# ekzhu/datasketch

Measured on AMD Instinct MI355X. Metric: MinHash signatures/sec (1M sets x 256 tokens, num_perm=128), higher is better.
Workload: dtype u64

## Files before the change

### datasketch_amd/csrc/mhx_internal.h

```cpp
#pragma once

#include <hip/hip_runtime.h>

#include <algorithm>
#include <cstdarg>
#include <cstdint>
#include <cstdio>
#include <mutex>
#include <string>
#include <unordered_map>

#include "mhx.h"

namespace mhx {

void set_error(const char *fmt, ...);
int fail(int code, const char *fmt, ...);
void forgive();

#define MHX_HIP_CHECK(expr)                                                                      \
    do {                                                                                         \
        hipError_t _e = (expr);                                                                  \
        if (_e != hipSuccess) {                                                                  \
            return ::mhx::fail(_e == hipErrorOutOfMemory ? MHX_ERR_OOM : MHX_ERR_HIP,            \
                               "%s failed: %s (%s:%d)", #expr, hipGetErrorString(_e), __FILE__,  \
                               __LINE__);                                                        \
        }                                                                                        \
    } while (0)

constexpr int kSigDigests = 2;
constexpr int kSigDigestsBM = 3;
constexpr int32_t kWeightedRows = -2;

constexpr unsigned int kPairListCap = 16384;
constexpr size_t kWorkBytes = 64 + sizeof(unsigned int) * kPairListCap;

#define MHX_GUARD(ctxp) std::lock_guard<std::recursive_mutex> _mhx_guard((ctxp)->mu)

#define MHX_REQUIRE(cond, ...)                                       \
    do {                                                             \
        if (!(cond)) return ::mhx::fail(MHX_ERR_INVALID, __VA_ARGS__); \
    } while (0)

hipError_t dev_malloc(void **p, size_t bytes, bool caller = false);
hipError_t dev_free(void *p);
bool guard_mode();

}

struct mhx_ctx {
    std::recursive_mutex mu;
    int device = 0;
    hipStream_t stream = nullptr;
    int num_cus = 0;
    int hw_cus = 0;
    int64_t lds_per_block = 64 << 10;
    int64_t hbm_bytes = 0;
    char name[128] = {0};
    void *scratch[5] = {nullptr, nullptr, nullptr, nullptr, nullptr};
    size_t scratch_bytes[5] = {0, 0, 0, 0, 0};
    int64_t opt_minhash_path = 0;
    int64_t opt_minhash_packed = 0;
    int64_t opt_minhash_adapt = 0;
    int64_t opt_minhash_share = 0;
    int64_t opt_minhash_p3 = 0;
    int64_t opt_minhash_ties = 0;
    int64_t opt_minhash_split = 0;
    int64_t opt_blocks_per_cu = 0;
    int64_t opt_debug_cus = 0;
    int64_t opt_minhash_prefetch = 1;
    int64_t opt_minhash_alias = -1;
    int64_t opt_weighted_path = 0;
    int64_t opt_weighted_min_dim = 0;
    int64_t opt_weighted_rescue = 0;
    int64_t opt_weighted_plan = 0;
    int64_t opt_weighted_kernel = 0;
    int64_t opt_weighted_debug = 0;
    int64_t opt_weighted_split = 0;
    int64_t opt_weighted_tail = 0;
    int64_t opt_weighted_direct = 0;
    int64_t opt_lsh_sort = 0;
    int64_t opt_lsh_gather = 0;
    int64_t opt_lsh_sort_bits = 0;
    int64_t opt_lsh_prehash = 0;
    int64_t opt_lsh_chunk = 0;
    int64_t opt_lsh_bigbins = 0;
    int64_t opt_lsh_team = 0;
    int64_t opt_lsh_merge_items = 0;
    int64_t opt_lsh_levels = 0;
    int64_t opt_pack_fused = 0;
    int64_t opt_weighted_refill = 0;
    int64_t opt_hll_split_tokens = 0;
    int64_t opt_bloom_lanes = 0;
    int64_t opt_jaccard_topk_path = 0;
    int64_t opt_jaccard_topk_segments = 0;
    int64_t opt_overlap_bins = 0;
    int64_t opt_host_chunk_bytes = 0;

    hipStream_t copy_in = nullptr;
    hipStream_t copy_out = nullptr;
    int ensure_copy_streams();

    unsigned long long *d_stats = nullptr;
    uint8_t *d_redo = nullptr;
    int64_t redo_capacity = 0;
    int64_t redo_sets = 0;
    int ensure_redo(int64_t n_sets);
    unsigned int *d_work = nullptr;
    int ensure_work();

    int ensure_scratch(int slot, size_t bytes);
    int activate() const;
};

struct mhx_perm {
    mhx_ctx *ctx = nullptr;
    int32_t num_perm = 0;
    uint64_t *d_a = nullptr;
    uint64_t *d_b = nullptr;
};

struct mhx_wgen {
    mhx_ctx *ctx = nullptr;
    int32_t sample_size = 0;
    int32_t dim = 0;
    float *d_params = nullptr;
    int32_t s_pad = 0;
    bool table_fast = false;
    float *d_aos = nullptr;
    float *d_walk_a = nullptr;
    uint32_t *d_walk_c = nullptr;
    void *d_walk_plan = nullptr;
    int plan_index = 0;
    bool walk_ok = false;
};

struct mhx_event {
    mhx_ctx *ctx = nullptr;
    hipEvent_t ev = nullptr;
};

namespace mhx {

int launch_minhash_bulk(mhx_perm *perm, const void *d_hv, int hv_dtype, const int64_t *d_offsets,
                        int64_t fixed_len, int64_t n_sets, int64_t total_tokens,
                        const uint64_t *d_init, int64_t init_stride, void *d_out, int out_dtype,
                        int64_t first_token = 0);
int launch_sha1_tokens(mhx_ctx *ctx, const uint8_t *d_bytes, const int64_t *d_offsets, int64_t n_tokens,
                       int out_dtype, void *d_out);
int launch_sha1_windows(mhx_ctx *ctx, const uint8_t *d_bytes, const int64_t *d_item_offsets, const int64_t *d_doc_offsets,
                        const int64_t *d_set_offsets, int64_t n_docs, int64_t n_windows, int64_t width, int out_dtype, void *d_out);
int launch_xxh_tokens(mhx_ctx *ctx, const uint8_t *d_bytes, const int64_t *d_offsets, int64_t n_tokens, int out_dtype, void *d_out);
int launch_xxh_windows(mhx_ctx *ctx, const uint8_t *d_bytes, const int64_t *d_item_offsets, const int64_t *d_doc_offsets,
                       const int64_t *d_set_offsets, int64_t n_docs, int64_t n_windows, int64_t width, int out_dtype, void *d_out);
int launch_words_count(mhx_ctx *ctx, const uint8_t *d_bytes, int64_t n_bytes, const int64_t *d_doc_offsets, int64_t n_docs,
                       const uint8_t *table, int64_t *n_words, int64_t *n_out_bytes);
int launch_words_emit(mhx_ctx *ctx, const uint8_t *d_bytes, int64_t n_bytes, const int64_t *d_doc_offsets, int64_t n_docs,
                      const uint8_t *table, uint8_t *d_out, int64_t *d_item_offsets, int64_t *d_word_doc_offsets);
int launch_minhash_merge(mhx_ctx *ctx, const uint64_t *d_x, const uint64_t *d_y, int64_t count,
                         uint64_t *d_out);
int launch_weighted(mhx_wgen *gen, const int64_t *d_indptr, const int32_t *d_indices,
                    const float *d_values, int values_are_logs, int64_t n_rows, int64_t nnz,
                    int64_t *d_out, uint8_t *d_nonempty);
int launch_weighted_log(mhx_ctx *ctx, const float *d_x, int64_t n, float *d_out);
int launch_wgen_transpose(mhx_wgen *gen, const float *d_rs, const float *d_lncs, const float *d_betas);
int launch_bbit_pack(mhx_ctx *ctx, const void *d_sig, int sig_dtype, int64_t n, int32_t k, int32_t b,
                     uint64_t *d_out);
int launch_band_keys(mhx_ctx *ctx, const uint64_t *d_sig, int64_t n, int32_t k, int32_t bands,
                     int32_t r, uint64_t *d_out);
int launch_band_digests(mhx_ctx *ctx, const void *d_sig, int sig_dtype, int64_t n, int32_t k, int32_t bands, int32_t r,
                        uint64_t *d_out, int layout = 0);
int launch_bbit_digest_fused(mhx_ctx *ctx, const void *d_sig, int sig_dtype, int64_t n, int32_t k, int32_t b, int32_t bands,
                             int32_t r, uint64_t *d_blocks, uint64_t *d_digests, int layout, bool *done);
int launch_jaccard_pairs(mhx_ctx *ctx, const void *d_a, const void *d_b, int sig_dtype, int32_t k, const int64_t *d_pairs,
                         int64_t m, int32_t *d_counts);
int launch_weighted_jaccard_pairs(mhx_ctx *ctx, const void *d_a, const void *d_b, int32_t samples, const int64_t *d_pairs, int64_t m,
                                  int32_t *d_counts);
int launch_weighted_dense(mhx_wgen *gen, const float *d_x, int values_are_logs, int64_t n_rows, int64_t *d_out,
                          uint8_t *d_nonempty);
int launch_lsh_candidate_pairs(mhx_ctx *ctx, const uint64_t *d_sorted_digests, const uint32_t *d_sorted_rows, int64_t n,
                               int32_t bands, int64_t *d_pairs, int64_t capacity, int64_t *n_pairs, int64_t *n_raw);
int launch_lsh_sort_bands(mhx_ctx *ctx, const void *d_sig, int sig_dtype, int64_t n, int32_t k, int32_t bands, int32_t r,
                          uint64_t *d_sorted_digests, uint32_t *d_sorted_rows);
int launch_lsh_query(mhx_ctx *ctx, const uint64_t *d_sorted_digests, const uint32_t *d_sorted_rows, int64_t n, int32_t bands,
                     int32_t r, const void *d_q_sig, const void *d_idx_sig, int sig_dtype, int32_t k, int64_t m,
                     int64_t *d_pairs, int64_t capacity, int64_t *n_pairs);
int launch_lsh_ensemble_query(mhx_ctx *ctx, const mhx_ensemble_level *levels, int32_t n_levels, const int64_t *start, int32_t n_parts,
                              const void *d_idx_sig, int sig_dtype, int32_t k, const void *d_q_sig, int64_t m, const uint8_t *d_choice,
// ... 69 lines not shown
```

### datasketch_amd/csrc/minhash_kernels.hip

```cpp
#include <type_traits>

#include "mhx_internal.h"

namespace mhx {
namespace {

constexpr uint64_t kMersenne = (1ull << 61) - 1;
constexpr uint32_t kMaxHash = 0xFFFFFFFFu;
constexpr int kWave = 64;

struct BulkArgs {
    const void *hv;
    const int64_t *offsets;
    int64_t fixed_len;
    int64_t n_sets;
    const uint64_t *a;
    const uint64_t *b;
    int32_t num_perm;
    int32_t path;
    unsigned long long *stats;
    uint8_t *redo;
    int32_t redo_match;
    unsigned int *sieve_hint;
    unsigned int *mode_word;
// ... 682 lines not shown
    const int lane = threadIdx.x & (kWave - 1);
    const TokT MHX_CONST_AS *hv = as_const(hv_vec);
    Perms<P> pm, pm_biased;
    bool active[P];
#pragma unroll
    for (int p = 0; p < P; ++p) {
        const int k = kbase + p * kWave + lane;
        active[p] = k < num_perm;
        const uint64_t av = active[p] ? a[k] : 0;
        pm.a_lo[p] = pm_biased.a_lo[p] = (uint32_t)av;
        pm.a_hi[p] = pm_biased.a_hi[p] = (uint32_t)(av >> 32);
        pm.b[p] = active[p] ? b[k] : 0;
        pm_biased.b[p] = pm.b[p] + 1;
    }
    Minima<P> res;
    bool redo = exact_only;
    if (!exact_only) {
        uint32_t acc[P];
#pragma unroll
        for (int p = 0; p < P; ++p) acc[p] = kMaxHash;
        hash_range<P, false, TokT>(hv, beg, end, pm_biased, acc);
        bool suspicious = false;
#pragma unroll
        for (int p = 0; p < P; ++p) {
            suspicious |= active[p] && acc[p] <= 7u;
            res.v[p] = acc[p] - 1u;
        }
        redo = __any(suspicious);
    }
    if (redo) {
        if (!exact_only && stats && lane == 0) atomicAdd(stats + 1, 1ull);
#pragma unroll
        for (int p = 0; p < P; ++p) res.v[p] = kMaxHash;
        hash_range<P, true, TokT>(hv, beg, end, pm, res.v);
    }
    return res;
}

template <int P, typename TokT, bool TAIL = true, bool TIES = false, bool SHARE = false, bool SHORT = true>
__device__ __forceinline__ bool sieve_minima(const TokT MHX_CONST_AS *hv, const TokT *hv_vec, int64_t beg,
                                             int64_t end, const Perms<P> &pm, const Perms<P> &pm_biased,
                                             const SievePerms<P> &sp, unsigned long long *stats, int lane,
                                             uint32_t *lds, uint32_t (&res)[P], bool *tied = nullptr) {
    const int64_t n = end - beg;
    const int nrows = (int)min(n / kRowTokens, (int64_t)(1 << 27));
#pragma unroll
    for (int p = 0; p < P; ++p) res[p] = kMaxHash;
    bool bad = false;
    if (nrows > 0) {
        int nblocks = 0;
        bad = sieve_range<P, TokT, TIES, SHARE, SHORT>(hv, hv_vec, beg, nrows, pm, sp, lds, lane, res, nblocks, tied);
        if (stats && lane == 0) atomicAdd(stats + 2, (unsigned long long)nblocks);
    }
    const int64_t tail = beg + (int64_t)nrows * kRowTokens;
    if (TAIL && tail < end) {
        uint32_t acc[P];
#pragma unroll
        for (int p = 0; p < P; ++p) acc[p] = kMaxHash;
        hash_range<P, false, TokT>(hv, tail, end, pm_biased, acc);
#pragma unroll
        for (int p = 0; p < P; ++p) {
            bad |= sp.active[p] && acc[p] <= 7u;
            res[p] = min(res[p], acc[p] - 1u);
        }
    }
    return __any(bad);
}

struct SieveBackoff {
    int skip = 0;
    int gap = 16;
    int streak = 0;
    __device__ __forceinline__ void failed() {
        if (++streak >= 2) {
            skip = gap;
            gap = min(2 * gap, 64);
        }
    }
    __device__ __forceinline__ void succeeded() {
        streak = 0;
        gap = 16;
    }
};

struct TiesBackoff {
    int skip = 0;
    int score = 0;
    __device__ __forceinline__ void failed() {
        score += 4;
        if (score >= 8) {
            skip = 32;
            score = 4;
        }
    }
    __device__ __forceinline__ void succeeded() { score = max(score - 1, 0); }
};

template <int P, typename TokT>
__device__ __forceinline__ void set_minima(const BulkArgs &args, const TokT MHX_CONST_AS *hv, const TokT *hv_vec,
                                           int64_t beg, int64_t end, const Perms<P> &pm,
                                           const Perms<P> &pm_biased, const SievePerms<P> &sp, int kbase,
                                           int lane, uint32_t *lds, SieveBackoff &bo, uint32_t (&res)[P]) {
    bool full = args.path != 0;
    if (!full) {
        if (bo.skip > 0) {
            --bo.skip;
            full = true;
        } else {
            full = sieve_minima<P, TokT>(hv, hv_vec, beg, end, pm, pm_biased, sp, args.stats, lane, lds, res);
            if (full) {
                if (args.stats && lane == 0) atomicAdd(args.stats, 1ull);
                bo.failed();
            } else {
                bo.succeeded();
            }
        }
    }
    if (full) {
        const Minima<P> m = full_minima<P, TokT>(hv_vec, beg, end, args.a, args.b, args.num_perm, kbase,
                                                 args.path == 1, args.stats);
#pragma unroll
        for (int p = 0; p < P; ++p) res[p] = m.v[p];
    }
}

template <int P, bool SHARE = false>
__device__ __forceinline__ void load_perms(const BulkArgs &args, int kbase, int lane, Perms<P> &pm,
                                           Perms<P> &pm_biased, SievePerms<P> &sp, int (&kidx)[P]) {
    uint32_t span = kWave;
    if constexpr (SHARE && P >= 3) {
        const int r = args.num_perm - (kbase + (P - 1) * kWave);
        span = r > 16 ? 32u : r > 8 ? 16u : r > 4 ? 8u : 4u;
    }
    sp.span = span;
#pragma unroll
    for (int p = 0; p < P; ++p) {
        const bool shared = SHARE && P >= 3 && p == P - 1;
        const int k = kbase + p * kWave + (shared ? lane & (int)(span - 1) : lane);
        const bool holds = k < args.num_perm;
        kidx[p] = holds && !(shared && lane >= (int)span) ? k : -1;
        const uint64_t a = holds ? args.a[k] : 0;
        pm.a_lo[p] = (uint32_t)a;
        pm.a_hi[p] = (uint32_t)(a >> 32);
        pm.b[p] = holds ? args.b[k] : 0;
        pm_biased.a_lo[p] = pm.a_lo[p];
        pm_biased.a_hi[p] = pm.a_hi[p];
        pm_biased.b[p] = pm.b[p] + 1;
        sp.a_lo[p] = pm.a_lo[p];
        sp.b8[p] = pm.b[p] + 8;
        sp.active[p] = kidx[p] >= 0;
    }
}

enum { MODE_SIEVE = 0, MODE_FULL = 1, MODE_DEDUP = 2, MODE_SIEVE_TIES = 3 };
enum { SHAPE_GENERAL = 0, SHAPE_PLAIN = 1, SHAPE_PLAIN_FIXED = 2, SHAPE_PLAIN_FIXED_ROWS = 3 };

template <int P, typename TokT, typename OutT, int MODE, int SHAPE, bool SHARE = false>
__global__ __launch_bounds__(256) void minhash_bulk_kernel(const BulkArgs args_in) {
    BulkArgs args = args_in;
    constexpr bool kSieve = MODE == MODE_SIEVE || MODE == MODE_SIEVE_TIES;
    constexpr bool kT32 = sizeof(TokT) == 4, kO32 = sizeof(OutT) == 4;
    constexpr bool kShortFold = !(MODE == MODE_DEDUP && P == 2 && kT32 && !kO32) &&
                                !(MODE == MODE_SIEVE_TIES && SHAPE == SHAPE_GENERAL && P == 4 && !kT32 && !kO32 && SHARE) &&
                                !(MODE == MODE_SIEVE_TIES && SHAPE == SHAPE_GENERAL && P == 1 && kT32 && kO32);
    if (kSieve && args.mode_word) {
        const unsigned int want_ties = *as_const(args.mode_word);
        if ((want_ties == 1u) != (MODE == MODE_SIEVE_TIES)) return;
    }
    if (MODE == MODE_FULL && args.mode_word && args.sieve_hint && blockIdx.x == 0 && threadIdx.x == 0) {
        const unsigned int t = __builtin_nontemporal_load(args.sieve_hint), f = __builtin_nontemporal_load(args.sieve_hint + 1);
        const unsigned int g = __builtin_nontemporal_load(args.sieve_hint + 2), m = *args.mode_word;
        const unsigned int tt = __builtin_nontemporal_load(args.sieve_hint + 3), tf = __builtin_nontemporal_load(args.sieve_hint + 5);
        if (t >= 64u) {
            const bool defeated = 4u * f > t;
            const bool heavy = m == 1u ? 5u * g > t : (tt >= 64u ? 5u * tf > tt : m == 2u);
            *args.mode_word = !defeated ? 0u : heavy ? 2u : 1u;
        }
    }
    if (SHAPE != SHAPE_GENERAL) {
        args.init = nullptr;
        args.init_stride = 0;
        args.stats = nullptr;
        args.alias_mask = -1;
    }
    if (SHAPE == SHAPE_PLAIN_FIXED || SHAPE == SHAPE_PLAIN_FIXED_ROWS) args.offsets = nullptr;
    const int lane = threadIdx.x & (kWave - 1);
    const int wave = __builtin_amdgcn_readfirstlane(threadIdx.x >> 6);
    const int waves_per_block = blockDim.x >> 6;
    const int kchunks = (args.num_perm + kWave * P - 1) / (kWave * P);
    constexpr int kLdsPerWave = MODE == MODE_DEDUP ? kDedupWordsPerWave : kStageWordsPerWave;
    __shared__ __attribute__((aligned(16))) uint32_t stage[4 * kLdsPerWave];
    uint32_t *lds = stage + wave * kLdsPerWave;
    Perms<P> pm, pm_biased;
    SievePerms<P> sp;
    int kidx[P];
    if (kSieve || MODE == MODE_DEDUP) load_perms<P, SHARE>(args, 0, lane, pm, pm_biased, sp, kidx);

    const TokT MHX_CONST_AS *hv = as_const(static_cast<const TokT *>(args.hv));
    const TokT *hv_vec = static_cast<const TokT *>(args.hv);
    const int64_t MHX_CONST_AS *offsets = as_const(args.offsets);
    OutT *__restrict__ out = static_cast<OutT *>(args.out);
    const int64_t stride = (int64_t)gridDim.x * waves_per_block;
    const bool flagged_only = !kSieve && args.redo != nullptr;
    unsigned int listed_n = 0;
    bool listed = false;
    if (MODE == MODE_FULL && flagged_only && args.pair_list) {
        listed_n = *as_const(args.pair_count);
        listed = listed_n <= kPairListCap;
    }
    const int64_t n_items = listed ? (int64_t)listed_n : flagged_only ? (args.n_sets + kWave - 1) / kWave * waves_per_block : args.n_sets;
    SieveBackoff backoff;
    TiesBackoff ties;
    int tried = 0, failed = 0, left = 0;
    if (MODE == MODE_SIEVE && args.sieve_hint) {
        const unsigned int t = __builtin_nontemporal_load(args.sieve_hint), f = __builtin_nontemporal_load(args.sieve_hint + 1);
        if (t >= 64u && 2u * f > t) {
            backoff.skip = 63;
            backoff.gap = 64;
            backoff.streak = 2;
        }
    }
    if (MODE == MODE_FULL && listed) {
        uint32_t *comb = stage;
        for (int64_t it = blockIdx.x; it < (int64_t)listed_n; it += gridDim.x) {
            const int64_t set = (int64_t)as_const(args.pair_list)[it];
            const int64_t beg = args.offsets ? offsets[set] : set * args.fixed_len;
            const int64_t end = args.offsets ? offsets[set + 1] : beg + args.fixed_len;
            const int64_t share = (end - beg + 31) / 32 * 8;
            const int64_t wbeg = min(end, beg + wave * share), wend = min(end, wbeg + share);
            for (int kc = 0; kc < kchunks; ++kc) {
                uint32_t mine[P];
#pragma unroll
                for (int p = 0; p < P; ++p) mine[p] = kMaxHash;
                if (wend > wbeg) {
                    const Minima<P> m = full_minima<P, TokT>(hv_vec, wbeg, wend, args.a, args.b, args.num_perm, kc * (kWave * P),
                                                             args.path == 1, args.stats);
#pragma unroll
                    for (int p = 0; p < P; ++p) mine[p] = m.v[p];
                }
#pragma unroll
                for (int p = 0; p < P; ++p) comb[(wave * P + p) * kWave + lane] = mine[p];
                __syncthreads();
                if (wave == 0) {
#pragma unroll
                    for (int p = 0; p < P; ++p) {
                        const int k = kc * (kWave * P) + p * kWave + lane;
                        if (k >= args.num_perm) continue;
                        uint32_t r = mine[p];
#pragma unroll
                        for (int w = 1; w < 4; ++w) r = min(r, comb[(w * P + p) * kWave + lane]);
                        uint64_t v = r;
                        if (args.init) {
                            const uint64_t iv = args.init[set * args.init_stride + k];
                            v = end > beg ? (uint64_t)min((iv >> 32) ? kMaxHash : (uint32_t)iv, r) : iv;
                        }
                        if (sizeof(OutT) == 4) v = v > kMaxHash ? kMaxHash : v;
                        out[set * args.num_perm + k] = (OutT)v;
                    }
                }
                __syncthreads();
            }
        }
        return;
    }
    for (int64_t item0 = (int64_t)blockIdx.x * waves_per_block + wave; item0 < n_items; item0 += stride) {
      const int64_t item = flagged_only ? item0 / waves_per_block : item0;
      unsigned long long todo = 1;
      if (flagged_only && !listed) {
          const int64_t cand = item * kWave + lane;
          const bool mine = (lane % waves_per_block) == (int)(item0 % waves_per_block);
          todo = __ballot(mine && cand < args.n_sets && args.redo[cand] == (uint8_t)args.redo_match);
      }
      while (todo) {
        const int bit = __builtin_ctzll(todo);
        todo &= todo - 1;
        const int64_t set = listed ? (int64_t)as_const(args.pair_list)[item0] : flagged_only ? item * kWave + bit : item;
        int64_t beg, end;
        if (args.offsets) {
            beg = offsets[set];
            end = offsets[set + 1];
        } else {
            beg = (args.alias_mask >= 0 ? (set & args.alias_mask) : set) * args.fixed_len;
            end = beg + args.fixed_len;
        }
        uint32_t warm = 0;
        {
            const int64_t nset = listed ? args.n_sets : flagged_only ? (todo ? item * kWave + __builtin_ctzll(todo) : args.n_sets) : item + stride;
            const bool skipping_on = MODE == MODE_SIEVE && backoff.skip > 1;
            if (args.prefetch && nset < args.n_sets && !skipping_on) {
                const int64_t nbeg = args.offsets ? offsets[nset] : nset * args.fixed_len;
                const int64_t nend = args.offsets ? offsets[nset + 1] : nbeg + args.fixed_len;
                const int64_t off = (int64_t)lane * 128;
                if (off < (nend - nbeg) * (int64_t)sizeof(TokT))
                    warm = *reinterpret_cast<const volatile uint32_t *>(reinterpret_cast<const char *>(args.hv) +
                                                                         nbeg * (int64_t)sizeof(TokT) + off);
            }
        }
        bool defer = false;
        if (MODE == MODE_SIEVE && end > beg && backoff.skip > 0) {
            --backoff.skip;
            defer = true;
        }
        for (int kc = 0; kc < kchunks && !defer; ++kc) {
            uint32_t res[P];
            if (kSieve) {
                if (kchunks > 1) load_perms<P, SHARE>(args, kc * (kWave * P), lane, pm, pm_biased, sp, kidx);
                if (end <= beg) {
#pragma unroll
                    for (int p = 0; p < P; ++p) res[p] = kMaxHash;
                } else {
                    bool tied = false;
                    defer = sieve_minima<P, TokT, SHAPE != SHAPE_PLAIN_FIXED_ROWS, MODE == MODE_SIEVE_TIES, SHARE, kShortFold>(hv, hv_vec, beg, end, pm, pm_biased, sp, args.stats, lane, lds, res,
                                                                                                          MODE == MODE_SIEVE_TIES ? &tied : nullptr);
                    if (kc == 0) ++tried;
                    if (MODE == MODE_SIEVE_TIES) {
                        if (defer || __any(tied)) ++failed;
                        if (defer) {
                            ++left;
                            break;
                        }
                    } else {
                        if (defer) {
                            ++failed;
                            backoff.failed();
                            break;
                        }
                        backoff.succeeded();
                    }
                }
            } else {
#pragma unroll
                for (int p = 0; p < P; ++p) {
                    const int k = kc * (kWave * P) + p * kWave + lane;
                    kidx[p] = k < args.num_perm ? k : -1;
                }
                if (end > beg) {
                    if (MODE == MODE_DEDUP) {
                        if (kchunks > 1) load_perms<P>(args, kc * (kWave * P), lane, pm, pm_biased, sp, kidx);
                        bool open = true;
                        if (!args.ties || (args.mode_word && *as_const(args.mode_word) == 1u)) {
                        } else if (ties.skip > 0) {
                            if (kc == kchunks - 1) --ties.skip;
                        } else {
                            open = sieve_minima<P, TokT, true, true, false, kShortFold>(hv, hv_vec, beg, end, pm, pm_biased, sp, nullptr, lane, lds, res);
                            if (kc == 0) ++tried, failed += open ? 1 : 0;
                            if (open) ties.failed(); else ties.succeeded();
                        }
                        if (open) {
#pragma unroll
                        for (int p = 0; p < P; ++p) res[p] = kMaxHash;
                        uint64_t cur[4];
                        load_quad<TokT>(hv_vec, beg, end, lane, cur);
                        defer = __any(dedup_sieve_range<P, TokT, kShortFold>(hv_vec, beg, end, pm, sp, lds, lane, cur, res));
                        if (defer) {
                            if (args.stats && lane == 0) atomicAdd(args.stats + 3, 1ull);
                            break;
                        }
                        }
                    } else {
                        const Minima<P> m = full_minima<P, TokT>(hv_vec, beg, end, args.a, args.b, args.num_perm,
                                                                 kc * (kWave * P), args.path == 1, args.stats);
#pragma unroll
                        for (int p = 0; p < P; ++p) res[p] = m.v[p];
                    }
                }
            }
#pragma unroll
            for (int p = 0; p < P; ++p) {
                if (kidx[p] < 0) continue;
                uint64_t v;
                if (args.init) {
                    const uint64_t iv = args.init[set * args.init_stride + kidx[p]];
                    if (end > beg) {
                        const uint32_t ic = (iv >> 32) ? kMaxHash : (uint32_t)iv;
                        v = min(ic, res[p]);
                    } else {
                        v = iv;
                    }
                } else {
                    v = (kSieve || end > beg) ? res[p] : kMaxHash;
                }
                if (sizeof(OutT) == 4) v = v > kMaxHash ? kMaxHash : v;
                char *row_out = reinterpret_cast<char *>(out + set * args.num_perm);
                *reinterpret_cast<OutT *>(row_out + (uint32_t)kidx[p] * (uint32_t)sizeof(OutT)) = (OutT)v;
            }
        }
        if (kSieve && lane == 0) {
            args.redo[set] = defer ? 1 : 0;
            if (defer && args.stats) atomicAdd(args.stats, 1ull);
        }
        if (MODE == MODE_DEDUP && defer && lane == 0) {
            args.redo[set] = 2;
            if (args.pair_list) {
                const unsigned int slot = atomicAdd(args.pair_count, 1u);
                if (slot < kPairListCap) args.pair_list[slot] = (unsigned int)set;
            }
        }
        asm volatile("" ::"v"(warm));
      }
    }
    if (kSieve && args.sieve_hint && lane == 0 && wave == 0 && (blockIdx.x & 15u) == 0 && tried > 0) {
        atomicAdd(args.sieve_hint, (unsigned int)tried);
        if (failed) atomicAdd(args.sieve_hint + 1, (unsigned int)failed);
        if (left) atomicAdd(args.sieve_hint + 2, (unsigned int)left);
    }
    if (MODE == MODE_DEDUP && args.sieve_hint && args.mode_word && lane == 0 && tried > 0) {
        atomicAdd(args.sieve_hint + 3, (unsigned int)tried);
        if (failed) atomicAdd(args.sieve_hint + 5, (unsigned int)failed);
    }
}

template <int KP, int P, typename TokT, typename OutT>
__global__ __launch_bounds__(256) void minhash_packed_kernel(const BulkArgs args) {
    constexpr int G = kWave / KP;
    constexpr int STRIDE = 36;
    const int lane = threadIdx.x & (kWave - 1);
    const int wave = __builtin_amdgcn_readfirstlane(threadIdx.x >> 6);
    const int g = lane / KP, k = lane % KP;
    __shared__ __attribute__((aligned(16))) uint32_t stage[4 * G * kStageWordsPerWave];
    uint32_t *tiles = stage + wave * (G * kStageWordsPerWave);
    uint32_t *my_tile = tiles + g * kStageWordsPerWave;
    Perms<P> pm;
    SievePerms<P> sp;
    bool any_active = false;
#pragma unroll
    for (int q = 0; q < P; ++q) {
        const bool active = k + q * KP < args.num_perm;
        const uint64_t a = active ? args.a[k + q * KP] : 0, b = active ? args.b[k + q * KP] : 0;
        pm.a_lo[q] = sp.a_lo[q] = (uint32_t)a;
        pm.a_hi[q] = (uint32_t)(a >> 32);
        pm.b[q] = b;
        sp.b8[q] = b + 8;
        sp.active[q] = active;
        any_active |= active;
    }
    const TokT *hv_vec = static_cast<const TokT *>(args.hv);
    OutT *__restrict__ out = static_cast<OutT *>(args.out);
    const unsigned long long group_lanes = (KP == 64 ? ~0ull : ((1ull << KP) - 1ull)) << (g * KP);
    const int64_t n_items = (args.n_sets + G - 1) / G;
    for (int64_t item = (int64_t)blockIdx.x * 4 + wave; item < n_items; item += (int64_t)gridDim.x * 4) {
        const int64_t set = item * G + g;
        const bool has = set < args.n_sets;
        int64_t beg = 0, end = 0;
        if (has) {
            beg = args.offsets ? args.offsets[set] : set * args.fixed_len;
            end = args.offsets ? args.offsets[set + 1] : beg + args.fixed_len;
        }
        uint32_t res[P];
#pragma unroll
        for (int q = 0; q < P; ++q) res[q] = kMaxHash;
        bool fail = false;
        for (int64_t boff = 0; __any(beg + boff < end); boff += kBlockRows * kRowTokens) {
            const int64_t blk = beg + boff;
            const int nb = (int)max((int64_t)0, min((int64_t)(kBlockRows * kRowTokens), end - blk));
#pragma unroll
            for (int j = 0; j < G; ++j) {
                const int jnb = __builtin_amdgcn_readlane(nb, j * KP);
                if (jnb == 0) continue;
                const uint32_t blo = __builtin_amdgcn_readlane((int)(uint32_t)blk, j * KP);
                const uint32_t bhi = __builtin_amdgcn_readlane((int)(uint32_t)((uint64_t)blk >> 32), j * KP);
                const int64_t jblk = (int64_t)(((uint64_t)bhi << 32) | blo);
                uint64_t t[4] = {0, 0, 0, 0};
                if (4 * lane + 3 < jnb) {
                    if constexpr (sizeof(TokT) == 8) {
                        const uint4 *src = reinterpret_cast<const uint4 *>(hv_vec + jblk + 4 * lane);
                        const uint4 lo = src[0], hi = src[1];
                        t[0] = ((uint64_t)lo.y << 32) | lo.x;
                        t[1] = ((uint64_t)lo.w << 32) | lo.z;
                        t[2] = ((uint64_t)hi.y << 32) | hi.x;
                        t[3] = ((uint64_t)hi.w << 32) | hi.z;
                    } else {
                        const uint4 v = *reinterpret_cast<const uint4 *>(hv_vec + jblk + 4 * lane);
                        t[0] = v.x;
                        t[1] = v.y;
                        t[2] = v.z;
                        t[3] = v.w;
                    }
                } else {
#pragma unroll
                    for (int i = 0; i < 4; ++i) t[i] = 4 * lane + i < jnb ? (uint64_t)hv_vec[jblk + 4 * lane + i] : 0;
                }
                uint4 *dst = reinterpret_cast<uint4 *>(tiles + j * kStageWordsPerWave + (lane >> 2) * STRIDE + (lane & 3) * 8);
                dst[0] = uint4{(uint32_t)t[0], (uint32_t)(t[0] >> 32), (uint32_t)t[1], (uint32_t)(t[1] >> 32)};
                dst[1] = uint4{(uint32_t)t[2], (uint32_t)(t[2] >> 32), (uint32_t)t[3], (uint32_t)(t[3] >> 32)};
            }
            const int nrows = nb >> 4, rest = nb & 15;
            Two rows[P];
            int max_rows = 0;
#pragma unroll
            for (int j = 0; j < G; ++j) max_rows = max(max_rows, __builtin_amdgcn_readlane(nrows, j * KP));
            for (int r = 0; r < max_rows; ++r) {
                const uint32_t *rowp = my_tile + r * STRIDE;
                uint32_t row[P];
#pragma unroll
                for (int c = 0; c < kRowTokens; c += 2) {
                    const uint32_t h0 = rowp[2 * c], h1 = rowp[2 * c + 2];
#pragma unroll
                    for (int q = 0; q < P; ++q) {
                        const uint32_t k0 = sieve_key(h0, sp.a_lo[q], sp.b8[q]);
                        const uint32_t k1 = sieve_key(h1, sp.a_lo[q], sp.b8[q]);
                        row[q] = c == 0 ? min(k0, k1) : umin3(row[q], k0, k1);
                    }
                }
#pragma unroll
                for (int q = 0; q < P; ++q) rows[q].add(r < nrows ? tag16(row[q], (uint32_t)r) : kMaxHash);
            }
            if (__any(rest > 0)) {
                uint32_t row[P];
#pragma unroll
                for (int q = 0; q < P; ++q) row[q] = kMaxHash;
                const uint32_t *rowp = my_tile + nrows * STRIDE;
                for (int c = 0; c < kRowTokens - 1; ++c) {
                    if (!__any(c < rest)) break;
                    const uint32_t h = rowp[2 * c];
#pragma unroll
                    for (int q = 0; q < P; ++q)
                        if (c < rest) row[q] = min(row[q], sieve_key(h, sp.a_lo[q], sp.b8[q]));
                }
#pragma unroll
                for (int q = 0; q < P; ++q)
                    if (rest > 0) rows[q].add(tag16(row[q], (uint32_t)nrows));
            }
            if (nb > 0) fail |= finish_block<P, STRIDE, 2, true>(rows, my_tile, pm, sp, res, (uint32_t)nrows, (uint32_t)rest);
        }
        const bool group_failed = (__ballot(fail && any_active) & group_lanes) != 0;
        if (has && k == 0) args.redo[set] = group_failed ? 1 : 0;
#pragma unroll
        for (int q = 0; q < P; ++q) {
            if (has && sp.active[q] && !group_failed) {
                uint64_t v;
                if (args.init) {
                    const uint64_t iv = args.init[set * args.init_stride + k + q * KP];
                    v = end > beg ? (uint64_t)min((iv >> 32) ? kMaxHash : (uint32_t)iv, res[q]) : iv;
                } else {
                    v = end > beg ? res[q] : kMaxHash;
                }
                if (sizeof(OutT) == 4) v = v > kMaxHash ? kMaxHash : v;
                out[set * args.num_perm + k + q * KP] = (OutT)v;
            }
        }
    }
}

template <typename OutT>
__global__ void minhash_fill_state_kernel(const BulkArgs args) {
    const int64_t total = args.n_sets * (int64_t)args.num_perm;
    OutT *__restrict__ out = static_cast<OutT *>(args.out);
    for (int64_t i = (int64_t)blockIdx.x * blockDim.x + threadIdx.x; i < total;
         i += (int64_t)gridDim.x * blockDim.x) {
        uint64_t v = kMaxHash;
        if (args.init) {
            const int64_t set = i / args.num_perm;
            v = args.init[set * args.init_stride + (i - set * args.num_perm)];
        }
        if (sizeof(OutT) == 4) v = v > kMaxHash ? kMaxHash : v;
        out[i] = (OutT)v;
    }
}

template <int P, typename TokT, typename OutT>
__global__ __launch_bounds__(256) void minhash_split_kernel(const BulkArgs args, int64_t first_token,
                                                            int64_t total_tokens, int64_t slice) {
    const int lane = threadIdx.x & (kWave - 1);
    const int wave = __builtin_amdgcn_readfirstlane(threadIdx.x >> 6);
    const int waves_per_block = blockDim.x >> 6;
    __shared__ __attribute__((aligned(16))) uint32_t stage[4 * kStageWordsPerWave];
    uint32_t *lds = stage + wave * kStageWordsPerWave;
    Perms<P> pm, pm_biased;
    SievePerms<P> sp;
    int kidx[P];
    load_perms<P>(args, blockIdx.y * (kWave * P), lane, pm, pm_biased, sp, kidx);
    const TokT MHX_CONST_AS *hv = as_const(static_cast<const TokT *>(args.hv));
    const TokT *hv_vec = static_cast<const TokT *>(args.hv);
    const int64_t MHX_CONST_AS *offsets = as_const(args.offsets);
    OutT *__restrict__ out = static_cast<OutT *>(args.out);

    const int64_t n_slices = (total_tokens + slice - 1) / slice;
    const int64_t stride = (int64_t)gridDim.x * waves_per_block;
    SieveBackoff backoff;
    for (int64_t s = (int64_t)blockIdx.x * waves_per_block + wave; s < n_slices; s += stride) {
        const int64_t s_beg = first_token + s * slice;
        const int64_t s_end = min(s_beg + slice, first_token + total_tokens);
        int64_t set;
        if (args.offsets) {
            int64_t lo = 0, hi = args.n_sets;
            while (hi - lo > 1) {
                const int64_t mid = (lo + hi) >> 1;
                if (offsets[mid] <= s_beg) lo = mid; else hi = mid;
            }
            set = lo;
        } else {
            set = s_beg / args.fixed_len;
        }
        for (; set < args.n_sets; ++set) {
            const int64_t set_beg = args.offsets ? offsets[set] : set * args.fixed_len;
            const int64_t set_end = args.offsets ? offsets[set + 1] : set_beg + args.fixed_len;
            if (set_beg >= s_end) break;
            const int64_t beg = max(set_beg, s_beg), end = min(set_end, s_end);
            if (end <= beg) continue;
            uint32_t res[P];
            set_minima<P, TokT>(args, hv, hv_vec, beg, end, pm, pm_biased, sp, blockIdx.y * (kWave * P), lane, lds, backoff, res);
#pragma unroll
            for (int p = 0; p < P; ++p) {
                if (kidx[p] < 0) continue;
                OutT *dst = out + set * args.num_perm + kidx[p];
                if (sizeof(OutT) == 8)
                    atomicMin(reinterpret_cast<unsigned long long *>(dst), (unsigned long long)res[p]);
                else
                    atomicMin(reinterpret_cast<unsigned int *>(dst), res[p]);
            }
        }
    }
}

__global__ void minhash_merge_kernel(const uint64_t *__restrict__ x, const uint64_t *__restrict__ y,
                                     int64_t count, uint64_t *__restrict__ out) {
    const int64_t n2 = count >> 1;
    const ulonglong2 *x2 = reinterpret_cast<const ulonglong2 *>(x);
    const ulonglong2 *y2 = reinterpret_cast<const ulonglong2 *>(y);
    ulonglong2 *o2 = reinterpret_cast<ulonglong2 *>(out);
    const int64_t stride = (int64_t)gridDim.x * blockDim.x;
    for (int64_t i = (int64_t)blockIdx.x * blockDim.x + threadIdx.x; i < n2; i += 4 * stride) {
        ulonglong2 xa[4], ya[4];
#pragma unroll
        for (int u = 0; u < 4; ++u) {
            if (i + u * stride < n2) {
                xa[u].x = __builtin_nontemporal_load(&x2[i + u * stride].x);
                xa[u].y = __builtin_nontemporal_load(&x2[i + u * stride].y);
                ya[u].x = __builtin_nontemporal_load(&y2[i + u * stride].x);
                ya[u].y = __builtin_nontemporal_load(&y2[i + u * stride].y);
            }
        }
#pragma unroll
        for (int u = 0; u < 4; ++u) {
            if (i + u * stride >= n2) break;
            ulonglong2 r;
            r.x = xa[u].x < ya[u].x ? xa[u].x : ya[u].x;
            r.y = xa[u].y < ya[u].y ? xa[u].y : ya[u].y;
            __builtin_nontemporal_store(r.x, &o2[i + u * stride].x);
            __builtin_nontemporal_store(r.y, &o2[i + u * stride].y);
        }
    }
    if ((count & 1) && blockIdx.x == 0 && threadIdx.x == 0)
        out[count - 1] = x[count - 1] < y[count - 1] ? x[count - 1] : y[count - 1];
}

unsigned resident_grid(mhx_ctx *ctx, const void *kernel, int64_t items) {
    int per_cu = 0;
    if (hipOccupancyMaxActiveBlocksPerMultiprocessor(&per_cu, kernel, 256, 0) != hipSuccess || per_cu < 1) {
        (void)hipGetLastError();
        per_cu = 2;
    }
    return (unsigned)std::max<int64_t>(1, std::min<int64_t>(items, (int64_t)ctx->num_cus * per_cu));
}

template <int P, typename TokT, typename OutT, int PF = P>
int launch_typed(mhx_ctx *ctx, const BulkArgs &args, int64_t first_token, int64_t total_tokens, bool split) {
    const int kchunks = (args.num_perm + kWave * P - 1) / (kWave * P);
    const int blocks_per_cu = ctx->opt_blocks_per_cu > 0 ? (int)ctx->opt_blocks_per_cu : (P >= 3 ? 128 : 64);
    const int64_t max_blocks = (int64_t)ctx->num_cus * blocks_per_cu;
    if (!split) {
        const int64_t want = (args.n_sets + 3) / 4;
        dim3 grid((unsigned)std::max<int64_t>(1, std::min(want, max_blocks)), 1u);
        if (args.path == 0) {
            if (int rc = ctx->ensure_work()) return rc;
            MHX_HIP_CHECK(hipMemsetAsync(ctx->d_work, 0, 8 * sizeof(unsigned int), ctx->stream));
            BulkArgs sieve_args = args;
            sieve_args.sieve_hint = ctx->d_work;
            sieve_args.mode_word = ctx->opt_minhash_adapt == 1 || args.stats ? nullptr : ctx->d_work + 8;
            const BulkArgs &args_s = sieve_args;
            const bool plain = !args.init && !args.stats && args.alias_mask < 0;
            const int np = args.num_perm;
            const bool packable = !args.stats && args.alias_mask < 0 && ctx->opt_minhash_packed != 1;
            const bool packed = packable && P <= 2 && (np <= 96 || (ctx->opt_minhash_packed == 2 && np <= 128));
            if (packed) {
                const int kp = np <= 8 ? 8 : np <= 16 ? 16 : np <= 32 ? 32 : np <= 64 ? 16 : np <= 96 ? 32 : 64;
                const int64_t items = (args.n_sets + 64 / kp - 1) / (64 / kp);
                dim3 pgrid((unsigned)std::max<int64_t>(1, std::min<int64_t>((items + 3) / 4, max_blocks)), 1u);
#define MHX_PACKED(KP_, P_) hipLaunchKernelGGL((minhash_packed_kernel<KP_, P_, TokT, OutT>), pgrid, dim3(256), 0, ctx->stream, args_s)
                if (np <= 8) MHX_PACKED(8, 1);
                else if (np <= 16) MHX_PACKED(16, 1);
                else if (np <= 32) MHX_PACKED(32, 1);
                else if (np <= 48) MHX_PACKED(16, 3);
                else if (np <= 64) MHX_PACKED(16, 4);
                else if (np <= 96) MHX_PACKED(32, 3);
                else MHX_PACKED(64, 2);
#undef MHX_PACKED
            } else {
            const bool fixed_rows = plain && !args.offsets && args.fixed_len % kRowTokens == 0;
            const int last_slot = args.num_perm - (P - 1) * kWave;
            const bool share = P >= 3 && kchunks == 1 && args.share_last && last_slot > 0 && last_slot <= 32;
            const auto first_launches = [&](auto share_tag) {
                constexpr bool SH = decltype(share_tag)::value;
#define MHX_SIEVE(MODE_, SHAPE_) hipLaunchKernelGGL((minhash_bulk_kernel<P, TokT, OutT, MODE_, SHAPE_, SH>), grid, dim3(256), 0, ctx->stream, args_s)
                if (fixed_rows) MHX_SIEVE(MODE_SIEVE, SHAPE_PLAIN_FIXED_ROWS);
                else if (plain && !args.offsets) MHX_SIEVE(MODE_SIEVE, SHAPE_PLAIN_FIXED);
                else if (plain) MHX_SIEVE(MODE_SIEVE, SHAPE_PLAIN);
                else MHX_SIEVE(MODE_SIEVE, SHAPE_GENERAL);
                if (args_s.mode_word) {
                    if (fixed_rows) MHX_SIEVE(MODE_SIEVE_TIES, SHAPE_PLAIN_FIXED_ROWS);
                    else MHX_SIEVE(MODE_SIEVE_TIES, SHAPE_GENERAL);
                }
#undef MHX_SIEVE
            };
            if constexpr (P >= 3) {
                if (share) first_launches(std::true_type());
                else first_launches(std::false_type());
            } else {
                (void)share;
                first_launches(std::false_type());
            }
            }
            const int64_t flag_groups = (args.n_sets + kWave - 1) / kWave;
            BulkArgs dedup = args;
            dedup.redo_match = 1;
            dedup.sieve_hint = sieve_args.sieve_hint;
            dedup.mode_word = packed ? nullptr : sieve_args.mode_word;
            if (args.n_sets <= 0xFFFFFFFFll) {
                dedup.pair_count = ctx->d_work + 4;
                dedup.pair_list = ctx->d_work + 16;
            }
            hipLaunchKernelGGL((minhash_bulk_kernel<PF, TokT, OutT, MODE_DEDUP, SHAPE_GENERAL>),
                               dim3(resident_grid(ctx, (const void *)minhash_bulk_kernel<PF, TokT, OutT, MODE_DEDUP, SHAPE_GENERAL>, flag_groups)),
                               dim3(256), 0, ctx->stream, dedup);
            BulkArgs rest = dedup;
            rest.redo_match = 2;
            hipLaunchKernelGGL((minhash_bulk_kernel<PF, TokT, OutT, MODE_FULL, SHAPE_GENERAL>),
                               dim3(resident_grid(ctx, (const void *)minhash_bulk_kernel<PF, TokT, OutT, MODE_FULL, SHAPE_GENERAL>, flag_groups)),
                               dim3(256), 0, ctx->stream, rest);
        } else {
            BulkArgs all = args;
            all.redo = nullptr;
            hipLaunchKernelGGL((minhash_bulk_kernel<PF, TokT, OutT, MODE_FULL, SHAPE_GENERAL>), grid, dim3(256), 0, ctx->stream, all);
        }
    } else {
        const int64_t total_out = args.n_sets * (int64_t)args.num_perm;
        const int64_t fill_blocks = std::max<int64_t>(1, std::min<int64_t>((total_out + 255) / 256, max_blocks));
        hipLaunchKernelGGL((minhash_fill_state_kernel<OutT>), dim3((unsigned)fill_blocks), dim3(256), 0,
                           ctx->stream, args);
        const int64_t waves = (int64_t)ctx->num_cus * 32;
        int64_t slice = (total_tokens + waves - 1) / waves;
        slice = slice > 128 ? (slice + 255) / 256 * 256 : std::max<int64_t>(64, (slice + 15) / 16 * 16);
        const int64_t n_slices = (total_tokens + slice - 1) / slice;
        const int64_t want = (n_slices + 3) / 4;
        dim3 grid((unsigned)std::max<int64_t>(1, std::min(want, max_blocks)), (unsigned)kchunks);
        hipLaunchKernelGGL((minhash_split_kernel<P, TokT, OutT>), grid, dim3(256), 0, ctx->stream, args,
                           first_token, total_tokens, slice);
    }
    MHX_HIP_CHECK(hipGetLastError());
    return MHX_OK;
}

template <typename TokT, typename OutT>
int launch_p(mhx_ctx *ctx, const BulkArgs &args, int64_t first_token, int64_t total_tokens, bool split) {
    if (args.num_perm <= 64) return launch_typed<1, TokT, OutT>(ctx, args, first_token, total_tokens, split);
    const auto slots = [&](int p) { return (args.num_perm + kWave * p - 1) / (kWave * p) * p; };
    const bool may3 = !split && ctx->opt_minhash_p3 != 1, may4 = !split && sizeof(TokT) == 8;
    int best = 2;
    if (may3 && slots(3) <= slots(best)) best = 3;
    if (may4 && slots(4) <= slots(best)) best = 4;
    if (best == 3) return launch_typed<3, TokT, OutT, 2>(ctx, args, first_token, total_tokens, split);
    if (best == 4) return launch_typed<4, TokT, OutT, 2>(ctx, args, first_token, total_tokens, split);
    return launch_typed<2, TokT, OutT>(ctx, args, first_token, total_tokens, split);
}

}

int launch_minhash_bulk(mhx_perm *perm, const void *d_hv, int hv_dtype, const int64_t *d_offsets,
                        int64_t fixed_len, int64_t n_sets, int64_t total_tokens,
                        const uint64_t *d_init, int64_t init_stride, void *d_out, int out_dtype, int64_t first_token) {
    mhx_ctx *ctx = perm->ctx;
    if (n_sets == 0) return MHX_OK;
    total_tokens -= first_token;
    BulkArgs args;
    args.hv = d_hv;
    args.offsets = d_offsets;
    args.fixed_len = fixed_len;
    args.n_sets = n_sets;
    args.a = perm->d_a;
    args.b = perm->d_b;
    args.num_perm = perm->num_perm;
    args.path = (int32_t)ctx->opt_minhash_path;
    args.stats = ctx->d_stats;
    args.redo = nullptr;
    args.redo_match = 1;
    args.sieve_hint = nullptr;
    args.mode_word = nullptr;
    args.alias_mask = ctx->opt_minhash_alias;
    args.pair_count = nullptr;
    args.pair_list = nullptr;
    args.prefetch = ctx->opt_minhash_prefetch == 2 || (ctx->opt_minhash_prefetch == 1 && (d_offsets != nullptr || fixed_len < 256));
    args.ties = ctx->opt_minhash_ties != 1;
    args.share_last = ctx->opt_minhash_share != 1;
    args.init = d_init;
    args.init_stride = init_stride;
    args.out = d_out;
    const int64_t waves_avail = (int64_t)ctx->num_cus * 16;
    bool split = n_sets < waves_avail && total_tokens > n_sets * 128 && total_tokens >= 1024;
    if (ctx->opt_minhash_split == 1) split = false;
    if (ctx->opt_minhash_split == 2) split = total_tokens > 0;
    ctx->redo_sets = 0;
    if (!split && args.path == 0) {
        if (int rc = ctx->ensure_redo(n_sets)) return rc;
        args.redo = ctx->d_redo;
        ctx->redo_sets = n_sets;
    }
    if (hv_dtype == MHX_U64 && out_dtype == MHX_U64) return launch_p<uint64_t, uint64_t>(ctx, args, first_token, total_tokens, split);
    if (hv_dtype == MHX_U64 && out_dtype == MHX_U32) return launch_p<uint64_t, uint32_t>(ctx, args, first_token, total_tokens, split);
    if (hv_dtype == MHX_U32 && out_dtype == MHX_U64) return launch_p<uint32_t, uint64_t>(ctx, args, first_token, total_tokens, split);
    if (hv_dtype == MHX_U32 && out_dtype == MHX_U32) return launch_p<uint32_t, uint32_t>(ctx, args, first_token, total_tokens, split);
    return fail(MHX_ERR_INVALID, "unknown hv_dtype/out_dtype (%d, %d)", hv_dtype, out_dtype);
}

int launch_minhash_merge(mhx_ctx *ctx, const uint64_t *d_x, const uint64_t *d_y, int64_t count,
                         uint64_t *d_out) {
    if (count == 0) return MHX_OK;
    const int64_t want = ((count >> 1) + 1023) / 1024;
    const int64_t blocks = std::max<int64_t>(1, std::min<int64_t>(want, (int64_t)ctx->num_cus * 32));
    hipLaunchKernelGGL(minhash_merge_kernel, dim3((unsigned)blocks), dim3(256), 0, ctx->stream, d_x, d_y,
                       count, d_out);
    MHX_HIP_CHECK(hipGetLastError());
    return MHX_OK;
}

}
```

Baseline: 519.3 million.

## Compact flagged sets into a list before dedup pass to skip redo-byte scanning

Adds a compaction kernel that runs after the sieve launches and uses wave ballots to collect the indices of sets flagged for redo into a bounded list in the work buffer. A new DEDUP_LIST mode of the bulk kernel walks that list directly instead of scanning every 64-set group's redo bytes, and it warms the first set's token cache lines. This targets the cost of the dedup pass sweeping all sets when few are flagged. In exchange it adds an extra kernel launch and atomics. It falls back to the old scan when the flag count exceeds the cap or full mode is selected.

```diff
diff --git a/datasketch_amd/csrc/mhx_internal.h b/datasketch_amd/csrc/mhx_internal.h
--- a/datasketch_amd/csrc/mhx_internal.h
+++ b/datasketch_amd/csrc/mhx_internal.h
@@ -33,7 +33,11 @@
 constexpr int32_t kWeightedRows = -2;
 
 constexpr unsigned int kPairListCap = 16384;
-constexpr size_t kWorkBytes = 64 + sizeof(unsigned int) * kPairListCap;
+constexpr unsigned int kFlagListCap = 16384;
+constexpr unsigned int kFlagCountWord = 6;
+constexpr unsigned int kFlagListWord = 16 + kPairListCap;
+constexpr unsigned int kNoFlagList = 0xFFFFFFFFu;
+constexpr size_t kWorkBytes = 64 + sizeof(unsigned int) * (kPairListCap + kFlagListCap);
 
 #define MHX_GUARD(ctxp) std::lock_guard<std::recursive_mutex> _mhx_guard((ctxp)->mu)
 
diff --git a/datasketch_amd/csrc/minhash_kernels.hip b/datasketch_amd/csrc/minhash_kernels.hip
--- a/datasketch_amd/csrc/minhash_kernels.hip
+++ b/datasketch_amd/csrc/minhash_kernels.hip
@@ -858,13 +858,39 @@
     }
 }
 
-enum { MODE_SIEVE = 0, MODE_FULL = 1, MODE_DEDUP = 2, MODE_SIEVE_TIES = 3 };
+enum { MODE_SIEVE = 0, MODE_FULL = 1, MODE_DEDUP = 2, MODE_SIEVE_TIES = 3, MODE_DEDUP_LIST = 4 };
 enum { SHAPE_GENERAL = 0, SHAPE_PLAIN = 1, SHAPE_PLAIN_FIXED = 2, SHAPE_PLAIN_FIXED_ROWS = 3 };
+
+__global__ __launch_bounds__(256) void minhash_flag_list_kernel(const BulkArgs args) {
+    unsigned int *count = args.sieve_hint + kFlagCountWord, *list = args.sieve_hint + kFlagListWord;
+    if (*as_const(args.mode_word) == 1u) {
+        if (blockIdx.x == 0 && threadIdx.x == 0) *count = kNoFlagList;
+        return;
+    }
+    const unsigned int t = __builtin_nontemporal_load(args.sieve_hint), f = __builtin_nontemporal_load(args.sieve_hint + 1);
+    if ((uint64_t)f * (uint64_t)args.n_sets > (uint64_t)kFlagListCap * t) {
+        if (blockIdx.x == 0 && threadIdx.x == 0) *count = kNoFlagList;
+        return;
+    }
+    const int lane = threadIdx.x & (kWave - 1);
+    const int64_t threads = (int64_t)gridDim.x * blockDim.x;
+    for (int64_t base = (int64_t)blockIdx.x * blockDim.x + (threadIdx.x - lane); base < args.n_sets; base += threads) {
+        const int64_t i = base + lane;
+        const bool flagged = i < args.n_sets && args.redo[i] == 1;
+        const unsigned long long m = __ballot(flagged);
+        if (!m) continue;
+        unsigned int slot = 0;
+        if (lane == __builtin_ctzll(m)) slot = atomicAdd(count, (unsigned int)__builtin_popcountll(m));
+        slot = __shfl(slot, __builtin_ctzll(m)) + (unsigned int)__builtin_popcountll(m & ((1ull << lane) - 1ull));
+        if (flagged && slot < kFlagListCap) list[slot] = (unsigned int)i;
+    }
+}
 
 template <int P, typename TokT, typename OutT, int MODE, int SHAPE, bool SHARE = false>
 __global__ __launch_bounds__(256) void minhash_bulk_kernel(const BulkArgs args_in) {
     BulkArgs args = args_in;
     constexpr bool kSieve = MODE == MODE_SIEVE || MODE == MODE_SIEVE_TIES;
+    constexpr bool kDedup = MODE == MODE_DEDUP || MODE == MODE_DEDUP_LIST;
     constexpr bool kT32 = sizeof(TokT) == 4, kO32 = sizeof(OutT) == 4;
     constexpr bool kShortFold = !(MODE == MODE_DEDUP && P == 2 && kT32 && !kO32) &&
                                 !(MODE == MODE_SIEVE_TIES && SHAPE == SHAPE_GENERAL && P == 4 && !kT32 && !kO32 && SHARE) &&
@@ -894,13 +920,13 @@
     const int wave = __builtin_amdgcn_readfirstlane(threadIdx.x >> 6);
     const int waves_per_block = blockDim.x >> 6;
     const int kchunks = (args.num_perm + kWave * P - 1) / (kWave * P);
-    constexpr int kLdsPerWave = MODE == MODE_DEDUP ? kDedupWordsPerWave : kStageWordsPerWave;
+    constexpr int kLdsPerWave = kDedup ? kDedupWordsPerWave : kStageWordsPerWave;
     __shared__ __attribute__((aligned(16))) uint32_t stage[4 * kLdsPerWave];
     uint32_t *lds = stage + wave * kLdsPerWave;
     Perms<P> pm, pm_biased;
     SievePerms<P> sp;
     int kidx[P];
-    if (kSieve || MODE == MODE_DEDUP) load_perms<P, SHARE>(args, 0, lane, pm, pm_biased, sp, kidx);
+    if (kSieve || kDedup) load_perms<P, SHARE>(args, 0, lane, pm, pm_biased, sp, kidx);
 
     const TokT MHX_CONST_AS *hv = as_const(static_cast<const TokT *>(args.hv));
     const TokT *hv_vec = static_cast<const TokT *>(args.hv);
@@ -914,7 +940,14 @@
         listed_n = *as_const(args.pair_count);
         listed = listed_n <= kPairListCap;
     }
-    const int64_t n_items = listed ? (int64_t)listed_n : flagged_only ? (args.n_sets + kWave - 1) / kWave * waves_per_block : args.n_sets;
+    const unsigned int MHX_CONST_AS *flist = as_const(args.sieve_hint + kFlagListWord);
+    unsigned int flist_n = 0;
+    bool flisted = false;
+    if (MODE == MODE_DEDUP_LIST) {
+        flist_n = *as_const(args.sieve_hint + kFlagCountWord);
+        flisted = flist_n <= kFlagListCap;
+    }
+    const int64_t n_items = listed ? (int64_t)listed_n : flisted ? (int64_t)flist_n : flagged_only ? (args.n_sets + kWave - 1) / kWave * waves_per_block : args.n_sets;
     SieveBackoff backoff;
     TiesBackoff ties;
     int tried = 0, failed = 0, left = 0;
@@ -969,10 +1002,15 @@
         }
         return;
     }
+    bool warmed = false;
     for (int64_t item0 = (int64_t)blockIdx.x * waves_per_block + wave; item0 < n_items; item0 += stride) {
-      const int64_t item = flagged_only ? item0 / waves_per_block : item0;
+      int64_t item = flagged_only ? item0 / waves_per_block : item0;
       unsigned long long todo = 1;
-      if (flagged_only && !listed) {
+      if (MODE == MODE_DEDUP_LIST && flisted) {
+          const unsigned int entry = flist[item0];
+          item = (int64_t)(entry / (unsigned int)kWave);
+          todo = 1ull << (entry % (unsigned int)kWave);
+      } else if (flagged_only && !listed) {
           const int64_t cand = item * kWave + lane;
           const bool mine = (lane % waves_per_block) == (int)(item0 % waves_per_block);
           todo = __ballot(mine && cand < args.n_sets && args.redo[cand] == (uint8_t)args.redo_match);
@@ -989,9 +1027,17 @@
             beg = (args.alias_mask >= 0 ? (set & args.alias_mask) : set) * args.fixed_len;
             end = beg + args.fixed_len;
         }
+        if (MODE == MODE_DEDUP_LIST && end > beg && !warmed) {
+            const int64_t off = (int64_t)lane * 128;
+            uint32_t own = 0;
+            if (off < (end - beg) * (int64_t)sizeof(TokT))
+                own = *reinterpret_cast<const volatile uint32_t *>(reinterpret_cast<const char *>(args.hv) + beg * (int64_t)sizeof(TokT) + off);
+            asm volatile("" ::"v"(own) : "memory");
+        }
         uint32_t warm = 0;
         {
             const int64_t nset = listed ? args.n_sets : flagged_only ? (todo ? item * kWave + __builtin_ctzll(todo) : args.n_sets) : item + stride;
+            if (MODE == MODE_DEDUP_LIST) warmed = args.prefetch && nset < args.n_sets;
             const bool skipping_on = MODE == MODE_SIEVE && backoff.skip > 1;
             if (args.prefetch && nset < args.n_sets && !skipping_on) {
                 const int64_t nbeg = args.offsets ? offsets[nset] : nset * args.fixed_len;
@@ -1041,7 +1087,7 @@
                     kidx[p] = k < args.num_perm ? k : -1;
                 }
                 if (end > beg) {
-                    if (MODE == MODE_DEDUP) {
+                    if (kDedup) {
                         if (kchunks > 1) load_perms<P>(args, kc * (kWave * P), lane, pm, pm_biased, sp, kidx);
                         bool open = true;
                         if (!args.ties || (args.mode_word && *as_const(args.mode_word) == 1u)) {
@@ -1095,7 +1141,7 @@
             args.redo[set] = defer ? 1 : 0;
             if (defer && args.stats) atomicAdd(args.stats, 1ull);
         }
-        if (MODE == MODE_DEDUP && defer && lane == 0) {
+        if (kDedup && defer && lane == 0) {
             args.redo[set] = 2;
             if (args.pair_list) {
                 const unsigned int slot = atomicAdd(args.pair_count, 1u);
@@ -1110,7 +1156,7 @@
         if (failed) atomicAdd(args.sieve_hint + 1, (unsigned int)failed);
         if (left) atomicAdd(args.sieve_hint + 2, (unsigned int)left);
     }
-    if (MODE == MODE_DEDUP && args.sieve_hint && args.mode_word && lane == 0 && tried > 0) {
+    if (kDedup && args.sieve_hint && args.mode_word && lane == 0 && tried > 0) {
         atomicAdd(args.sieve_hint + 3, (unsigned int)tried);
         if (failed) atomicAdd(args.sieve_hint + 5, (unsigned int)failed);
     }
@@ -1416,6 +1462,10 @@
                 (void)share;
                 first_launches(std::false_type());
             }
+            if (args_s.mode_word && args.n_sets <= 0xFFFFFFFFll) {
+                const int64_t list_blocks = std::min<int64_t>((args.n_sets + 255) / 256, (int64_t)ctx->num_cus * 8);
+                hipLaunchKernelGGL(minhash_flag_list_kernel, dim3((unsigned)list_blocks), dim3(256), 0, ctx->stream, args_s);
+            }
             }
             const int64_t flag_groups = (args.n_sets + kWave - 1) / kWave;
             BulkArgs dedup = args;
@@ -1426,9 +1476,14 @@
                 dedup.pair_count = ctx->d_work + 4;
                 dedup.pair_list = ctx->d_work + 16;
             }
-            hipLaunchKernelGGL((minhash_bulk_kernel<PF, TokT, OutT, MODE_DEDUP, SHAPE_GENERAL>),
-                               dim3(resident_grid(ctx, (const void *)minhash_bulk_kernel<PF, TokT, OutT, MODE_DEDUP, SHAPE_GENERAL>, flag_groups)),
-                               dim3(256), 0, ctx->stream, dedup);
+            if (dedup.mode_word && dedup.pair_list)
+                hipLaunchKernelGGL((minhash_bulk_kernel<PF, TokT, OutT, MODE_DEDUP_LIST, SHAPE_GENERAL>),
+                                   dim3(resident_grid(ctx, (const void *)minhash_bulk_kernel<PF, TokT, OutT, MODE_DEDUP_LIST, SHAPE_GENERAL>, flag_groups)),
+                                   dim3(256), 0, ctx->stream, dedup);
+            else
+                hipLaunchKernelGGL((minhash_bulk_kernel<PF, TokT, OutT, MODE_DEDUP, SHAPE_GENERAL>),
+                                   dim3(resident_grid(ctx, (const void *)minhash_bulk_kernel<PF, TokT, OutT, MODE_DEDUP, SHAPE_GENERAL>, flag_groups)),
+                                   dim3(256), 0, ctx->stream, dedup);
             BulkArgs rest = dedup;
             rest.redo_match = 2;
             hipLaunchKernelGGL((minhash_bulk_kernel<PF, TokT, OutT, MODE_FULL, SHAPE_GENERAL>),
```

Result: no change. 524.1 million (median of 6 runs) (+0.9%).
